# fabioiuri/DRecPy

Hardware: AMD Instinct MI355X
Metric: training samples/sec (user-item pairs) (higher is better)
Workload: dtype f32; 1 GPU; CDAE hidden_factors=128 sampled-output sparse-Adagrad on synth-10m-shaped synthetic (10000000 users x 1000000 items, 199573906 positives), corruption 0.2, neg_ratio 5; batch_per_gpu=65536, global_batch=65536, touch_list=prepared ahead on a side stream, batches=fresh device-sampled batch every step (sampler running ahead on the side stream)

## Files before the change

drecpy_amd/_lib.py:

```python
import ctypes as C
import os

_HERE = os.path.dirname(os.path.abspath(__file__))
LIB_PATH = os.path.join(_HERE, 'libdrx.so')

LOSS_BCE, LOSS_MSE = 0, 1
TARGETS_REFERENCE, TARGETS_PER_ROW = 0, 1
OPT_ADAM, OPT_ADAGRAD, OPT_ROWWISE_ADAGRAD = 0, 1, 2
DENSE_AUX_CLEAN = 0x100
KEY_NONE = 0xFFFFFFFF
SHARD_SELF_BYPASS = 1
BATCH_SHARE_USERS = 1


class DrxError(RuntimeError):
    pass


DRX_REC_SIGMOID_BIAS, DRX_REC_BIAS, DRX_REC_CLIP = 0, 1, 2

KNN_METRICS = {'cosine': 0, 'adjusted_cosine': 1, 'cosine_cf': 2, 'jaccard': 3, 'msd': 4, 'pearson': 5}
KNN_USER, KNN_ITEM = 0, 1
KNN_AGGREGATIONS = {'mean': 0, 'weighted_mean': 1}

# ... 269 lines not shown
    'drx_sampler_create': (C.c_void_p, [C.c_void_p, C.c_void_p, C.c_void_p, C.c_int64, C.c_int32, C.c_int32,
                                        C.c_double, C.c_int64]),
    'drx_sampler_sample': (C.c_int, [C.c_void_p, C.c_int32, C.c_void_p, C.c_void_p, C.c_void_p]),
    'drx_cdae_reference_draw': (C.c_int, [C.c_void_p, C.c_void_p, C.c_void_p, C.c_int64, C.c_uint64, C.c_void_p, C.c_void_p, C.c_int32,
                                          C.c_int32, C.c_double, C.c_void_p, C.c_void_p, C.c_void_p, C.c_void_p, C.c_void_p, C.c_void_p,
                                          C.c_int64]),
    'drx_drawahead_create': (C.c_void_p, [C.c_void_p, C.c_void_p, C.c_void_p, C.c_void_p, C.c_void_p, C.c_int32]),
    'drx_drawahead_submit': (C.c_int64, [C.c_void_p, C.c_int32, C.c_int64, C.c_uint64, C.c_int32, C.c_double, C.c_void_p, C.c_void_p,
                                         C.c_void_p, C.c_void_p, C.c_void_p, C.c_void_p, C.c_int64]),
    'drx_drawahead_wait': (C.c_int, [C.c_void_p, C.c_int32, C.c_int64]),
    'drx_drawahead_destroy': (None, [C.c_void_p]),
    'drx_cdae_fit_slot_bytes': (C.c_size_t, [C.c_int32, C.c_int64]),
    'drx_cdae_fit_dense': (C.c_int, [C.POINTER(CdaeParams), C.POINTER(Optim), C.POINTER(History), C.c_void_p, C.c_void_p, C.c_int32,
                                     C.c_float, C.c_int64, C.c_int32, C.c_int32, C.c_int64, C.c_void_p, C.c_void_p, C.c_size_t,
                                     C.c_int32, C.c_void_p, C.c_size_t, C.c_void_p, C.c_size_t, C.c_void_p]),
    'drx_sampler_draw': (C.c_int, [C.c_void_p, C.c_int32, C.c_int32, C.c_void_p, C.c_void_p, C.c_void_p, C.c_void_p]),
    'drx_sampler_destroy': (None, [C.c_void_p]),
    'drx_cdae_kshard_forward': (C.c_int, [C.POINTER(CdaeParams), C.POINTER(History), C.POINTER(Batch), C.c_void_p, C.c_void_p,
                                          C.c_void_p]),
    'drx_cdae_kshard_forward_prepared': (C.c_int, [C.POINTER(CdaeParams), C.POINTER(History), C.POINTER(Batch), C.c_void_p, C.c_size_t, C.c_void_p,
                                                   C.c_void_p, C.c_void_p]),
    'drx_cdae_kshard_step': (C.c_int, [C.POINTER(CdaeParams), C.POINTER(Optim), C.POINTER(History), C.POINTER(Batch), C.c_int32,
                                       C.c_void_p, C.c_void_p, C.c_void_p, C.c_size_t, C.c_void_p, C.c_size_t, C.c_void_p,
                                       C.c_void_p, C.c_void_p]),
    'drx_cdae_prep_result_bytes': (C.c_size_t, [C.POINTER(CdaeParams), C.c_int32, C.c_int32]),
    'drx_cdae_prep_part_out_bytes': (C.c_size_t, [C.POINTER(CdaeParams), C.c_int32, C.c_int32, C.c_int32]),
    'drx_cdae_prep_part_layout': (C.c_int, [C.POINTER(CdaeParams), C.c_int32, C.c_int32, C.c_int32, C.POINTER(C.c_size_t)]),
    'drx_cdae_prep_part_bytes': (C.c_size_t, [C.POINTER(CdaeParams), C.c_int32, C.c_int32, C.c_int32]),
    'drx_cdae_sparse_prepare_part': (C.c_int, [C.POINTER(CdaeParams), C.POINTER(History), C.POINTER(Batch), C.c_int32, C.c_int32,
                                               C.c_void_p, C.c_size_t, C.c_void_p, C.c_size_t, C.c_void_p]),
    'drx_cdae_sparse_prepare_assemble': (C.c_int, [C.POINTER(CdaeParams), C.POINTER(Batch), C.c_void_p, C.c_int32, C.c_void_p,
                                                   C.c_size_t, C.c_void_p, C.c_void_p]),
    'drx_sort_pairs_temp_bytes': (C.c_size_t, [C.c_int64, C.c_int32]),
    'drx_sort_pairs': (C.c_int, [C.c_void_p, C.c_void_p, C.c_void_p, C.c_void_p, C.c_int64, C.c_int32, C.c_void_p, C.c_size_t, C.c_void_p]),
    'drx_list_sampler_create': (C.c_void_p, [C.c_void_p, C.c_void_p, C.c_void_p, C.c_int32, C.c_int32, C.c_int32, C.c_int32,
                                             C.c_int32, C.c_int32, C.c_int64]),
    'drx_list_sampler_sample': (C.c_int, [C.c_void_p, C.c_int32, C.c_void_p, C.c_void_p, C.c_void_p, C.c_int64, C.c_void_p,
                                          C.c_void_p, C.c_int64, C.c_void_p, C.c_void_p, C.c_int64]),
    'drx_list_sampler_last_hint': (C.c_int32, [C.c_void_p]),
    'drx_list_sampler_destroy': (None, [C.c_void_p]),
    'drx_rng_create': (C.c_void_p, [C.c_int64]),
    'drx_rng_destroy': (None, [C.c_void_p]),
    'drx_rng_random': (C.c_double, [C.c_void_p]),
    'drx_rng_randint': (C.c_int64, [C.c_void_p, C.c_int64, C.c_int64]),
    'drx_rng_discard': (None, [C.c_void_p, C.c_uint64]),
    'drx_rng_corruption_keep': (C.c_int, [C.c_void_p, C.c_void_p, C.c_void_p, C.c_int32, C.c_void_p, C.c_int32,
                                          C.c_double, C.c_void_p, C.c_void_p, C.c_int64]),
}


def batch_offsets(indptr, ids):
    import torch
    B = int(ids.numel())
    off = torch.empty(B + 1, dtype=torch.int32, device=ids.device)
    need = int(lib().drx_point_sample_scratch_bytes(B))
    sc = torch.empty(need, dtype=torch.uint8, device=ids.device)
    check(lib().drx_batch_offsets(ptr(indptr), ptr(ids), B, ptr(off), ptr(sc), need, stream_ptr(ids.device)), 'drx_batch_offsets')
    return off


def sumsq(tensors, device=None):
    import torch
    ts = [t for t in tensors if t is not None and t.numel()]
    if not ts:
        return 0.0
    dev = ts[0].device
# ... 49 lines not shown
```

drecpy_amd/csrc/drx_prep.hpp:

```cpp
#pragma once
#include <algorithm>
#include "drx_common.hpp"
#include "drx_rows.hpp"
#include "drx_segreduce.hpp"
#include "drx_scan.hpp"

namespace drx {

struct WireGeo {
  int ipr, cshift, world;
  __host__ __device__ __forceinline__ uint32_t wire(int item, int is_out) const {
    const int o = item / ipr;
    const uint32_t l = 2u * (uint32_t)(item - o * ipr) + (uint32_t)(is_out ? 1 : 0);
    return (((l >> cshift) * (uint32_t)world + (uint32_t)o) << cshift) | (l & ((1u << cshift) - 1u));
  }
  __host__ __device__ __forceinline__ uint32_t local(uint32_t w) const {
    return (((w >> cshift) / (uint32_t)world) << cshift) | (w & ((1u << cshift) - 1u));
  }
  __host__ __device__ __forceinline__ uint32_t unit(uint32_t w) const { return w >> cshift; }
};

struct TouchPresence {
  uint8_t *present;
  WireGeo G;
  __device__ __forceinline__ uint32_t wire(int item, int is_out) const { return G.wire(item, is_out); }
};

#ifndef DRX_HOT_LDS_LOOKUP
#define DRX_HOT_LDS_LOOKUP 1
#endif
struct HotMark {
  const int16_t *slot;
  uint32_t *mask;
  int H, Bw;
  const int32_t *item;
  int tbits;
};
static inline int hot_table_bits(int H) {
  int b = 0;
  while ((1 << b) < 4 * H) ++b;
  return b;
}
static inline size_t hot_table_lds_bytes(int H) { return H > 0 && DRX_HOT_LDS_LOOKUP ? ((size_t)6 << hot_table_bits(H)) : 0; }
__device__ __forceinline__ uint32_t hot_table_home(int item, int tbits) { return ((uint32_t)item * 2654435761u) >> (32 - tbits); }

static __global__ __launch_bounds__(kBlock) void k_sparse_touches(int n_items, DrxHistory H, DrxBatch bt, uint32_t qthr, uint32_t *keys,
                                                           uint32_t *vals, int T, uint8_t *solo, uint32_t *zero_a,
                                                           int n_zero_a, uint32_t *zero_b, int n_zero_b, uint32_t *zero_c, int n_zero_c,
                                                           TouchPresence pres, HotMark hot) {
  constexpr int G = 16;
  const int lane = threadIdx.x % G;
  const int b = blockIdx.x * (kBlock / G) + threadIdx.x / G;
  for (int w = blockIdx.x * kBlock + threadIdx.x; w < n_zero_a; w += gridDim.x * kBlock) zero_a[w] = 0u;
  for (int w = blockIdx.x * kBlock + threadIdx.x; w < n_zero_b; w += gridDim.x * kBlock) zero_b[w] = 0u;
  for (int w = blockIdx.x * kBlock + threadIdx.x; w < n_zero_c; w += gridDim.x * kBlock) zero_c[w] = 0u;
  __shared__ uint32_t hm[DRX_MAX_HOT];
  extern __shared__ __align__(16) int hot_table[];
  const uint32_t tmask = (1u << hot.tbits) - 1u;
  uint16_t *const hot_slot_of = reinterpret_cast<uint16_t *>(hot_table + tmask + 1);
  if (hot.slot) {
    for (int i = threadIdx.x; i < hot.H; i += kBlock) hm[i] = 0u;
    if (DRX_HOT_LDS_LOOKUP) {
      for (int i = threadIdx.x; i <= (int)tmask; i += kBlock) hot_table[i] = -1;
      __syncthreads();
      for (int i = threadIdx.x; i < hot.H; i += kBlock) {
        const int it = hot.item[i];
        uint32_t at = hot_table_home(it, hot.tbits);
        while (atomicCAS(&hot_table[at], -1, it) != -1) at = (at + 1u) & tmask;
        hot_slot_of[at] = (uint16_t)i;
      }
    }
    __syncthreads();
  }
  if (b < bt.B) {
  if (solo && lane == 0) { solo[b] = 0; solo[bt.B + b] = 0; }
  if (b == bt.B - 1)
    for (int j = bt.keep_off[bt.B] + 2 * bt.B + lane; j < T; j += G) { keys[j] = DRX_KEY_NONE; vals[j] = 0; }
  const int u = bt.uid[b];
  const int64_t s = H.indptr[u], e = H.indptr[u + 1];
  const int base = bt.keep_off[b] + 2 * b;
  const uint8_t *kp = bt.keep ? bt.keep + bt.keep_off[b] : nullptr;
  for (int64_t j = s + lane; j < e; j += G) {
    const uint32_t jj = (uint32_t)(j - s);
    const bool kf = kp ? (kp[jj] != 0) : (hash_u32(bt.mask_seed, (uint32_t)b, jj) >= qthr);
    const int item = H.indices[j];
    int hs = -1;
    if (hot.slot && kf) {
      if (DRX_HOT_LDS_LOOKUP) {
        for (uint32_t at = hot_table_home(item, hot.tbits);; at = (at + 1u) & tmask) {
          const int k = hot_table[at];
          if (k == item) hs = (int)hot_slot_of[at];
          if (k == item || k == -1) break;
        }
      } else hs = (int)hot.slot[item];
    }
    keys[base + jj] = kf && hs < 0 ? (uint32_t)item : DRX_KEY_NONE;
    vals[base + jj] = (uint32_t)b;
    if (hs >= 0) atomicOr(&hm[hs], 1u << (b & 15));
    if (pres.present && kf) pres.present[pres.wire(item, 0)] = 1;
  }
  if (lane == 0) {
    const int deg = (int)(e - s);
    keys[base + deg] = (uint32_t)(n_items + bt.iid[b]);       vals[base + deg] = (uint32_t)b;
    if (pres.present) pres.present[pres.wire(bt.iid[b], 1)] = 1;
    keys[base + deg + 1] = (uint32_t)(2 * n_items) + (uint32_t)u;       vals[base + deg + 1] = (uint32_t)b;
  }
  }
  if (hot.slot) {
    __syncthreads();
    uint16_t *const m16 = reinterpret_cast<uint16_t *>(hot.mask);
    const size_t row = 2 * (size_t)hot.Bw;
    const bool tail = blockIdx.x + 1 == gridDim.x && blockIdx.x + 1 < row;
    for (int i = threadIdx.x; i < hot.H; i += kBlock) {
      m16[(size_t)i * row + blockIdx.x] = (uint16_t)hm[i];
      if (tail) m16[(size_t)i * row + blockIdx.x + 1] = 0;
    }
  }
}

static __global__ __launch_bounds__(1024) void k_degree_counts(const int32_t *__restrict__ keep_off, int B, unsigned int *__restrict__ work) {
  __shared__ unsigned int cnt[256];
  degree_counts_body<1024>(keep_off, B, work, (int)blockIdx.x, cnt);
}

template <int NT>
__device__ __forceinline__ void degree_scatter_body(const int32_t *__restrict__ keep_off, int B, unsigned int *__restrict__ work,
                                                    int32_t *__restrict__ order, int block_id, unsigned int *lds ) {
  unsigned int *start = lds, *cnt = lds + 256, *base = lds + 512;
  for (int i = threadIdx.x; i < 256; i += NT) cnt[i] = 0;
  if (threadIdx.x < 64) {
    unsigned int c[4], sum = 0;
#pragma unroll
    for (int q = 0; q < 4; ++q) { c[q] = work[threadIdx.x * 4 + q]; sum += c[q]; }
    unsigned int inc = sum;
#pragma unroll
    for (int o = 1; o < 64; o <<= 1) { const unsigned int t = __shfl_up(inc, o); if ((int)threadIdx.x >= o) inc += t; }
    unsigned int run = inc - sum;
#pragma unroll
    for (int q = 0; q < 4; ++q) { start[threadIdx.x * 4 + q] = run; run += c[q]; }
  }
  __syncthreads();
  const int b = block_id * NT + (int)threadIdx.x, lane = threadIdx.x & 63;
  const bool valid = b < B;
  const int d = valid ? degree_bucket(keep_off, b) : 0;
  const unsigned long long m = same_bucket_lanes(valid, d);
  const int leader = valid ? __ffsll((long long)m) - 1 : lane;
  unsigned int at = 0;
  if (valid && lane == leader) at = atomicAdd(&cnt[d], (unsigned int)__popcll(m));
// ... 478 lines not shown
                     R.order_work, 512);
  int rc = sort_pairs(stemp, sb, k2, ks, v2, vs, (size_t)2 * B, bits2, st);
  if (rc) return rc;
  hipLaunchKernelGGL(k_tp_runs, dim3((2 * B + 255) / 256 < 1024 ? (2 * B + 255) / 256 : 1024), dim3(256), 0, st, ks, 2 * B, start, end);
  const int egrid = U < (1 << 20) ? U : (1 << 20);
  const int wgrid = (int)((nnz + 255) / 256 < 16384 ? (nnz + 255) / 256 : 16384);
  const int rt = share_item_triples(p->ld);
  if (share) {
    const int ig = (B + 255) / 256;
    hipLaunchKernelGGL(k_tp_item_flags, dim3(ig), dim3(256), 0, st, ks, B, rt, start, R.pitem, R.n_du);
    rc = scan_i32(sctemp2, scb2, R.pitem, R.pitem, (size_t)B, true, st);
    if (rc) return rc;
    hipLaunchKernelGGL(k_tp_item_finish, dim3(ig), dim3(256), 0, st, ks, vs, B, rt, start, end, hist->indptr, R.usamp, R.pitem, R.witem,
                       R.n_du, R.plan.cnt);
    hipLaunchKernelGGL(k_tp_item_order, dim3(ig), dim3(256), 0, st, ks, B, rt, start, hist->indptr, R.pitem, R.worder, R.n_du);
    hipLaunchKernelGGL((k_tp_count<true>), dim3(egrid), dim3(256), 0, st, *hist, *bt, qthr, U, start, end, vs, cnt, km, rt);
  } else
    hipLaunchKernelGGL((k_tp_count<false>), dim3(egrid), dim3(256), 0, st, *hist, *bt, qthr, U, start, end, vs, cnt, km, rt);
  int *cnt_last = (int *)R.vals;
  DRX_HIP(hipMemcpyAsync(cnt_last, cnt + (nnz - 1), sizeof(int), hipMemcpyDeviceToDevice, st));
  rc = scan_i32(sctemp, scb, cnt, cnt, (size_t)nnz, false, st);
  if (rc) return rc;
  if (share)
    hipLaunchKernelGGL((k_tp_write<true>), dim3(wgrid), dim3(256), 0, st, *hist, *bt, qthr, start, end, vs, cnt, km, R.keys_s, R.vals_s, R.pitem, rt, row_end);
  else
    hipLaunchKernelGGL((k_tp_write<false>), dim3(wgrid), dim3(256), 0, st, *hist, *bt, qthr, start, end, vs, cnt, km, R.keys_s, R.vals_s, R.pitem, rt, row_end);
  hipLaunchKernelGGL(k_tp_tail, dim3(2048), dim3(256), 0, st, ks, vs, B, U, N, cnt + (nnz - 1), cnt_last, R.T, R.keys_s, R.vals_s, R.plan.cnt);
  return DRX_OK;
}

static int prepare_impl(const DrxCdaeParams *p, const DrxHistory *hist, const DrxBatch *bt, const PrepBufs &R, hipStream_t st,
                        bool with_marks = false, TouchPresence pres = TouchPresence{nullptr, WireGeo{1, 0, 1}},
                        const int16_t *hot_slot = nullptr, const int32_t *hot_item = nullptr) {
  const int gpb = kBlock / 16;
  if (R.H > 0 && (!hot_slot || !hot_item || !hot_list_fits(R.T, *p, pres.present != nullptr))) return DRX_EINVAL;
  if (hist->t_rank && hist->t_users && hist->t_pos && hist->t_items && !pres.present && long_segments(R.T, *p)) {
    const int32_t *row_end = nullptr;
    const int rc = prepare_transposed(p, hist, bt, R, st, with_marks, &row_end);
    if (rc == DRX_OK) {
      PrepBufs Rb = R;
      Rb.plan.row_end = row_end;
      Rb.plan.row_end_keys = (uint32_t)p->n_items;
      if (with_marks && p->ld > 16) {
        if (!share_users(p, hist, bt, R)) order_by_degree(bt, R, st, true);
        const int blocks = std::max(2048, (R.n_chunks + 255) / 256);
        hipLaunchKernelGGL(k_plan_and_mark, dim3(blocks), dim3(256), 0, st, R.keys_s, R.vals_s, R.T, R.n_chunks,
                           kSegBlock / pick_geom(p->ld).G, Rb.plan, (uint32_t)p->n_items, bt->B, R.solo_v, R.solo_o, 0, bt->keep_off,
                           R.order_work, R.order);
        if (R.plan.xrank) hipLaunchKernelGGL(k_place_blocks, dim3(256), dim3(256), 0, st, Rb.plan, R.n_chunks);
        return DRX_OK;
      }
      return plan_spans(p, bt, Rb, st, true);
    }
    if (rc != kTpFallback) return rc;
  }
  uint32_t *sort_zero = nullptr;
  size_t sort_zero_words = 0;
  sort_pairs_zero_region(R.sort_temp, (size_t)R.T, R.bits, &sort_zero, &sort_zero_words);
  hipLaunchKernelGGL(k_sparse_touches, dim3((bt->B + gpb - 1) / gpb), dim3(kBlock), hot_table_lds_bytes(R.H), st, p->n_items, *hist, *bt,
                     q_threshold(bt->q), R.keys, R.vals, R.T, R.solo_v, R.plan.cnt, plan_zero_words(R), R.order_work, 512,
                     sort_zero, (int)sort_zero_words, pres, HotMark{R.H > 0 ? hot_slot : nullptr, R.hmask, R.H, R.Bw, hot_item, hot_table_bits(R.H)});
  const bool fused_order = with_marks && p->ld > 16;
  const SortRider rider{fused_order ? bt->keep_off : nullptr, bt->B, R.order_work};
  const int rc = sort_pairs_ex(R.sort_temp, R.sort_bytes, R.keys, R.keys_s, R.vals, R.vals_s, (size_t)R.T, R.bits, true, st, true, rider);
  if (rc) return rc;
  if (with_marks && p->ld > 16) {
    const int blocks = std::max(2048, (R.n_chunks + 255) / 256);
    const int order_blocks = (bt->B + 255) / 256;
    hipLaunchKernelGGL(k_plan_and_mark, dim3(blocks + order_blocks), dim3(256), 0, st, R.keys_s, R.vals_s, R.T, R.n_chunks,
                       kSegBlock / pick_geom(p->ld).G, R.plan, (uint32_t)p->n_items, bt->B, R.solo_v, R.solo_o,
                       order_blocks, bt->keep_off, R.order_work, R.order);
    if (R.plan.xrank) hipLaunchKernelGGL(k_place_blocks, dim3(256), dim3(256), 0, st, R.plan, R.n_chunks);
    return DRX_OK;
  }
  return plan_spans(p, bt, R, st, true);
}

static int mark_solo(const DrxCdaeParams *p, const DrxBatch *bt, const PrepBufs &R, hipStream_t st, bool cleared) {
  if (!cleared) {
    DRX_HIP(hipMemsetAsync(R.solo_v, 0, (size_t)bt->B * 2, st));
  }
  if (p->ld <= 16) return DRX_OK;
  hipLaunchKernelGGL(k_mark_solo, dim3(2048), dim3(256), 0, st, R.keys_s, R.vals_s, R.T, (uint32_t)p->n_items, bt->B, R.solo_v,
                     R.solo_o);
  return DRX_OK;
}


}
```

drecpy_amd/csrc/drx_sort.hip:

```cpp
#include <cstdlib>
#include <cstring>
#include <hip/hip_runtime.h>
#include "drx_common.hpp"

namespace drx {

#ifndef DRX_SORT_THREADS
#define DRX_SORT_THREADS 512
#endif
#ifndef DRX_SORT_IPT
#define DRX_SORT_IPT 16
#endif
constexpr int kSortThreads = DRX_SORT_THREADS;
constexpr int kSortWaves = kSortThreads / 64;
constexpr int kSortIPT = DRX_SORT_IPT;
constexpr int kSortTile = kSortThreads * kSortIPT;
constexpr int kMaxPasses = 4;
constexpr uint32_t kStAgg = 1u << 30, kStIncl = 2u << 30, kCountMask = (1u << 30) - 1;
constexpr int kDropNone = 1, kFirstPass = 2, kLastPass = 4;

struct SortPlan {
  int passes;
  int rbits[kMaxPasses];
  int shift[kMaxPasses];
};

inline SortPlan sort_plan(int bits) {
  SortPlan p{};
  int passes = (bits + 10) / 11;
  if (bits <= 8) passes = 1;
  int r = (bits + passes - 1) / passes;
  if (r < 8 && bits >= 8) r = 8;
  if (r <= 8) r = 8; else if (r <= 10) r = 10; else r = 11;
  p.passes = (bits + r - 1) / r;
  for (int i = 0; i < p.passes; ++i) { p.rbits[i] = r; p.shift[i] = i * r; }
  return p;
}

struct SortLayout {
  uint32_t *tmp_k, *tmp_v;
  uint32_t *hist;
  uint32_t *ticket;
  uint32_t *desc;
  size_t zero_begin, zero_bytes;
  size_t total;
  int tiles;
};

inline SortLayout sort_layout(void *temp, size_t n, const SortPlan &P) {
  SortLayout L{};
  Carver cv(temp, (size_t)-1);
  L.tiles = (int)((n + kSortTile - 1) / kSortTile);
  if (P.passes >= 2) { L.tmp_k = cv.take<uint32_t>(n); L.tmp_v = cv.take<uint32_t>(n); }
  cv.off = align_up(cv.off, 256);
  L.zero_begin = cv.off;
  L.hist = cv.take<uint32_t>((size_t)kMaxPasses * 2048);
  L.ticket = cv.take<uint32_t>(64);
  size_t d = 0;
  for (int i = 0; i < P.passes; ++i) d += (size_t)L.tiles << P.rbits[i];
  L.desc = cv.take<uint32_t>(d);
  L.zero_bytes = cv.off - L.zero_begin;
  L.total = align_up(cv.off, 256);
  return L;
}

__global__ __launch_bounds__(512) void k_digit_histograms(const uint32_t *__restrict__ keys, size_t n, SortPlan P, uint32_t *__restrict__ hist,
                                                          int drop_none, SortRider rider, int rider_blocks) {
  __shared__ uint32_t h[kMaxPasses * 2048];
  if ((int)blockIdx.x >= (int)gridDim.x - rider_blocks) {
    degree_counts_body<512>(rider.keep_off, rider.B, rider.counts, (int)blockIdx.x - ((int)gridDim.x - rider_blocks), h);
    return;
  }
  const size_t hist_threads = (size_t)((int)gridDim.x - rider_blocks) * blockDim.x;
  for (int i = threadIdx.x; i < P.passes * 2048; i += blockDim.x) h[i] = 0;
  __syncthreads();
  const uint32_t lane = threadIdx.x & 63;
  for (size_t i = (size_t)blockIdx.x * blockDim.x + threadIdx.x; i < n; i += hist_threads) {
    const uint32_t k = keys[i];
    if (drop_none && k == DRX_KEY_NONE) continue;
    for (int p = 0; p < P.passes; ++p) {
      const uint32_t rep_bits = 11u - (uint32_t)P.rbits[p];
      const uint32_t d = (k >> P.shift[p]) & ((1u << P.rbits[p]) - 1);
      atomicAdd(&h[p * 2048 + (d << rep_bits) + (lane & ((1u << rep_bits) - 1u))], 1u);
    }
  }
  __syncthreads();
  for (int p = 0; p < P.passes; ++p) {
    const uint32_t rep_bits = 11u - (uint32_t)P.rbits[p], reps = 1u << rep_bits;
    for (uint32_t d = threadIdx.x; d < (1u << P.rbits[p]); d += blockDim.x) {
      uint32_t c = 0;
      for (uint32_t r = 0; r < reps; ++r) c += h[p * 2048 + (d << rep_bits) + r];
      if (c) atomicAdd(&hist[p * 2048 + d], c);
    }
  }
}

template <int R>
__global__ __launch_bounds__(kSortThreads) void k_onesweep_pass(const uint32_t *__restrict__ kin, const uint32_t *__restrict__ vin,
                                                               uint32_t *__restrict__ kout, uint32_t *__restrict__ vout, size_t n, int shift,
                                                               const uint32_t *__restrict__ ghist, uint32_t *ticket, uint32_t *desc, uint32_t n_tiles,
                                                               int flags, uint32_t *next_hist, int next_shift) {
  constexpr int RADIX = 1 << R;
  constexpr int BPT = (RADIX + kSortThreads - 1) / kSortThreads;
  extern __shared__ __align__(16) uint32_t sort_lds[];
  uint32_t (*whist)[RADIX] = reinterpret_cast<uint32_t (*)[RADIX]>(sort_lds);
  uint32_t *gbase = sort_lds + kSortWaves * RADIX;
  uint32_t *lstart = gbase + RADIX;
  uint32_t *skey = lstart + RADIX, *sval = skey + kSortTile;
  constexpr int REPB = 11 - R, REP = 1 << REPB;
  uint32_t *nh = sval + kSortTile;
  __shared__ uint32_t s_tile, s_tile_valid;
  __shared__ uint32_t wl[kSortWaves], wg[kSortWaves];
  const int tid = threadIdx.x, lane = tid & 63, w = tid >> 6;
  const bool drop = flags & kDropNone, first = flags & kFirstPass, last = flags & kLastPass;
  size_t n_valid = n;
  if (drop) {
    uint32_t part = 0;
    for (int d = tid; d < RADIX; d += kSortThreads) part += ghist[d];
#pragma unroll
    for (int o = 32; o > 0; o >>= 1) part += __shfl_xor(part, o);
    if (lane == 0) wl[w] = part;
    __syncthreads();
    uint32_t tot = 0;
    for (int ww = 0; ww < kSortWaves; ++ww) tot += wl[ww];
    n_valid = tot;
    __syncthreads();
// ... 72 lines not shown
    __syncthreads();
#pragma unroll
    for (int q = 0; q < BPT; ++q) { const int d = tid * BPT + q; if (d < RADIX) local[q] = lstart[d]; sl += local[q]; }
    __syncthreads();
    uint32_t il = sl, ig = sg;
#pragma unroll
    for (int o = 1; o < 64; o <<= 1) {
      const uint32_t tl = __shfl_up(il, o), tg = __shfl_up(ig, o);
      if (lane >= o) { il += tl; ig += tg; }
    }
    if (lane == 63) { wl[w] = il; wg[w] = ig; }
    __syncthreads();
    uint32_t ol = il - sl, og = ig - sg;
    for (int ww = 0; ww < w; ++ww) { ol += wl[ww]; og += wg[ww]; }
#pragma unroll
    for (int q = 0; q < BPT; ++q) {
      const int d = tid * BPT + q;
      if (d < RADIX) { lstart[d] = ol; gbase[d] = og; }
      ol += local[q]; og += glob[q];
      if (d == RADIX - 1) s_tile_valid = ol;
    }
  }
  __syncthreads();

#pragma unroll
  for (int q = 0; q < BPT; ++q) {
    const int d = tid + q * kSortThreads;
    excl[q] = 0;
    if (d < RADIX && tile > 0) {
      uint32_t sum = 0;
      int p = (int)tile - 1;
      bool done = false;
      while (!done) {
        uint32_t wv[8];
#pragma unroll
        for (int u = 0; u < 8; ++u)
          wv[u] = (p - u >= 0) ? __hip_atomic_load(desc + ((size_t)(p - u) << R) + d, __ATOMIC_RELAXED, __HIP_MEMORY_SCOPE_AGENT) : kStIncl;
#pragma unroll
        for (int u = 0; u < 8; ++u) {
          if (done) break;
          uint32_t x = wv[u];
          while ((x >> 30) == 0) {
            __builtin_amdgcn_s_sleep(1);
            x = __hip_atomic_load(desc + ((size_t)(p - u) << R) + d, __ATOMIC_RELAXED, __HIP_MEMORY_SCOPE_AGENT);
          }
          sum += x & kCountMask;
          if ((x >> 30) == 2u) done = true;
        }
        p -= 8;
      }
      excl[q] = sum;
      __hip_atomic_store(desc + ((size_t)tile << R) + d, kStIncl | (sum + cnt[q]), __ATOMIC_RELAXED, __HIP_MEMORY_SCOPE_AGENT);
    }
  }
#pragma unroll
  for (int q = 0; q < BPT; ++q) {
    const int d = tid + q * kSortThreads;
    if (d < RADIX) gbase[d] = gbase[d] + excl[q] - lstart[d];
  }
#pragma unroll
  for (int it = 0; it < kSortIPT; ++it) {
    const int idx = w * (64 * kSortIPT) + it * 64 + lane;
    if (idx < tile_n && !(drop && key[it] == DRX_KEY_NONE)) {
      const uint32_t d = (key[it] >> shift) & (RADIX - 1);
      const uint32_t pos = lstart[d] + whist[w][d] + pre[it];
      skey[pos] = key[it];
      sval[pos] = val[it];
    }
  }
  __syncthreads();
  const int tile_out = (int)s_tile_valid;
  for (int i = tid; i < tile_out; i += kSortThreads) {
    const uint32_t k = skey[i];
    const uint32_t d = (k >> shift) & (RADIX - 1);
    const size_t o = (size_t)gbase[d] + (size_t)i;
    kout[o] = k;
    vout[o] = sval[i];
  }
  }
  if (next_hist) {
    for (int d = tid; d < RADIX; d += kSortThreads) {
      uint32_t c = 0;
// ... 17 lines not shown
static int launch_pass(const uint32_t *sk, const uint32_t *sv, uint32_t *dk, uint32_t *dv, size_t n, int shift, const uint32_t *gh, uint32_t *ticket,
                       uint32_t *desc, int tiles, int flags, uint32_t *next_hist, int next_shift, hipStream_t stream) {
  const size_t lds = onesweep_lds_bytes(R);
  if (lds > 48 * 1024) DRX_HIP(hipFuncSetAttribute((const void *)k_onesweep_pass<R>, hipFuncAttributeMaxDynamicSharedMemorySize, (int)lds));
  hipLaunchKernelGGL(k_onesweep_pass<R>, dim3(tiles < sort_grid() ? tiles : sort_grid()), dim3(kSortThreads), lds, stream, sk, sv, dk, dv, n, shift, gh,
                     ticket, desc, (uint32_t)tiles, flags, next_hist, next_shift);
  return 0;
}

size_t sort_pairs_temp_bytes(size_t n, int end_bit) {
  const SortPlan P = sort_plan(end_bit);
  return sort_layout(nullptr, n ? n : 1, P).total + 256;
}

void sort_pairs_zero_region(void *temp, size_t n, int end_bit, uint32_t **words, size_t *n_words) {
  const SortPlan P = sort_plan(end_bit);
  char *t = (char *)align_up((size_t)temp, 256);
  const SortLayout L = sort_layout(t, n ? n : 1, P);
  *words = (uint32_t *)(t + L.zero_begin);
  *n_words = L.zero_bytes / 4;
}

int sort_pairs_ex(void *temp, size_t temp_bytes, const uint32_t *kin, uint32_t *kout, const uint32_t *vin, uint32_t *vout, size_t n, int end_bit,
                  bool drop_none, hipStream_t stream, bool pre_zeroed, SortRider rider) {
  if (n == 0) return 0;
  if (n >= (1u << 30)) return DRX_EINVAL;
  const SortPlan P = sort_plan(end_bit);
  char *t = (char *)align_up((size_t)temp, 256);
  const SortLayout L = sort_layout(t, n, P);
  if ((size_t)(t - (char *)temp) + L.total > temp_bytes) return DRX_ESCRATCH;
  if (!pre_zeroed) DRX_HIP(hipMemsetAsync(t + L.zero_begin, 0, L.zero_bytes, stream));
  int hgrid = (int)((n + 8 * 512 - 1) / (8 * 512));
  if (hgrid > sort_grid()) hgrid = sort_grid();
  SortPlan P1 = P;
  P1.passes = 1;
  const int rider_blocks = rider.keep_off ? (rider.B + 511) / 512 : 0;
  hipLaunchKernelGGL(k_digit_histograms, dim3(hgrid + rider_blocks), dim3(512), 0, stream, kin, n, P1, L.hist, drop_none ? 1 : 0, rider,
                     rider_blocks);
  const uint32_t *src_k = kin, *src_v = vin;
  uint32_t *desc = L.desc;
  for (int p = 0; p < P.passes; ++p) {
    const bool to_out = ((P.passes - 1 - p) & 1) == 0;
    uint32_t *dk = to_out ? kout : L.tmp_k, *dv = to_out ? vout : L.tmp_v;
    const uint32_t *gh = L.hist + (size_t)p * 2048;
    const int flags = (drop_none ? kDropNone : 0) | (p == 0 ? kFirstPass : 0) | (p == P.passes - 1 ? kLastPass : 0);
    int rc;
    uint32_t *nh = p + 1 < P.passes ? L.hist + (size_t)(p + 1) * 2048 : nullptr;
    const int ns = p + 1 < P.passes ? P.shift[p + 1] : 0;
    if (P.rbits[p] == 8) rc = launch_pass<8>(src_k, src_v, dk, dv, n, P.shift[p], gh, L.ticket + p, desc, L.tiles, flags, nh, ns, stream);
    else if (P.rbits[p] == 10) rc = launch_pass<10>(src_k, src_v, dk, dv, n, P.shift[p], gh, L.ticket + p, desc, L.tiles, flags, nh, ns, stream);
    else rc = launch_pass<11>(src_k, src_v, dk, dv, n, P.shift[p], gh, L.ticket + p, desc, L.tiles, flags, nh, ns, stream);
    if (rc) return rc;
    desc += (size_t)L.tiles << P.rbits[p];
    src_k = dk; src_v = dv;
  }
  DRX_LAUNCH_CHECK();
  return 0;
}

int sort_pairs(void *temp, size_t temp_bytes, const uint32_t *kin, uint32_t *kout, const uint32_t *vin,
               uint32_t *vout, size_t n, int end_bit, hipStream_t stream) {
  return sort_pairs_ex(temp, temp_bytes, kin, kout, vin, vout, n, end_bit, false, stream);
}

}

extern "C" {
size_t drx_sort_pairs_temp_bytes(int64_t n, int32_t key_bits) {
  if (n < 0 || key_bits < 1 || key_bits > 32) return 0;
  return drx::sort_pairs_temp_bytes((size_t)n, key_bits) + 256;
}
int drx_sort_pairs(const uint32_t *keys_in, uint32_t *keys_out, const uint32_t *vals_in, uint32_t *vals_out, int64_t n, int32_t key_bits,
                   void *temp, size_t temp_bytes, void *stream) {
  if (n < 0 || key_bits < 1 || key_bits > 32 || (n > 0 && (!keys_in || !keys_out || !vals_in || !vals_out || !temp))) return DRX_EINVAL;
  return drx::sort_pairs(temp, temp_bytes, keys_in, keys_out, vals_in, vals_out, (size_t)n, key_bits, (hipStream_t)stream);
}
}
```

include/drx.h:

```cpp
#ifndef DRX_H_
#define DRX_H_

#include <stddef.h>
#include <stdint.h>

#ifdef __cplusplus
extern "C" {
#endif

#define DRX_VERSION 100

enum {
  DRX_OK = 0,
  DRX_EINVAL = -1,
  DRX_ESCRATCH = -2,
  DRX_ENOTIMPL = -3,
  DRX_ERETRY = -4,
  DRX_ECOMM = -5
};

#define DRX_MAX_K 1024
#define DRX_KEY_NONE 0xFFFFFFFFu

enum { DRX_LOSS_BCE = 0, DRX_LOSS_MSE = 1 };
// ... 400 lines not shown

int drx_rows_pair_scores(const float *table, const float *bias, int32_t n_rows, int32_t ld, int32_t epilogue,
                         const float *q, int32_t n_q, const int32_t *q_row, const int32_t *t_row, int64_t P,
                         float *out_score, void *stream);

#define DRX_KNN_COSINE          0
#define DRX_KNN_ADJUSTED_COSINE 1
#define DRX_KNN_COSINE_CF       2
#define DRX_KNN_JACCARD         3
#define DRX_KNN_MSD             4
#define DRX_KNN_PEARSON         5
#define DRX_KNN_USER            0
#define DRX_KNN_ITEM            1
#define DRX_KNN_MEAN            0
#define DRX_KNN_WEIGHTED_MEAN   1
size_t drx_knn_neighbours_scratch_bytes(int32_t R, int32_t C, int32_t k, int32_t splits);
int drx_knn_neighbours(const int64_t *indptr, const int32_t *indices, const float *values, int64_t nnz, int32_t R, int32_t C,
                       int32_t metric, int32_t k, int32_t m, double shrinkage, double max_diff, int32_t splits,
                       int32_t *out_idx, float *out_sim, void *scratch, size_t scratch_bytes, void *stream);

int drx_knn_row_means(const int64_t *indptr, const float *values, int64_t nnz, int32_t R, double *out_mean, void *stream);

size_t drx_knn_score_rows_scratch_bytes(int32_t type, int32_t R, int32_t n_items);
int drx_knn_score_rows(int32_t type, int32_t aggregation, const int64_t *indptr, const int32_t *indices, const float *values, int64_t nnz,
                       int32_t n_users, int32_t n_items, const int32_t *nb_idx, const float *nb_sim, int32_t k,
                       const int32_t *uid, int32_t R, const double *fallback, float *out, uint32_t *cand_mask,
                       void *scratch, size_t scratch_bytes, void *stream);
int drx_knn_pair_scores(int32_t type, int32_t aggregation, const int64_t *indptr, const int32_t *indices, const float *values, int64_t nnz,
                        int32_t n_users, int32_t n_items, const int32_t *nb_idx, const float *nb_sim, int32_t k,
                        const int32_t *uid, const int32_t *iid, int64_t P, const double *fallback, double *out, uint8_t *none,
                        void *stream);

size_t drx_sort_pairs_temp_bytes(int64_t n, int32_t key_bits);
int drx_sort_pairs(const uint32_t *keys_in, uint32_t *keys_out, const uint32_t *vals_in, uint32_t *vals_out, int64_t n, int32_t key_bits,
                   void *temp, size_t temp_bytes, void *stream);

size_t drx_idmap_scratch_bytes(int64_t n);
int drx_idmap_build(const int64_t *raw, int64_t n, int32_t *codes, int64_t *uniques,
                    int32_t *n_unique, void *scratch, size_t scratch_bytes, void *stream);

typedef struct DrxSampler DrxSampler;
DrxSampler *drx_sampler_create(const int32_t *h_uid, const int32_t *h_iid, const double *h_val, int64_t n_rows,
                               int32_t neg_ratio, int32_t has_threshold, double threshold, int64_t seed);
int drx_sampler_sample(DrxSampler *s, int32_t n, int32_t *h_uid_out, int32_t *h_iid_out, double *h_val_out);
enum { DRX_DRAW_MIXED = 0, DRX_DRAW_NEGATIVE = 1, DRX_DRAW_POSITIVE = 2 };
int drx_sampler_draw(DrxSampler *s, int32_t kind, int32_t n, int32_t *h_uid_out, int32_t *h_iid_out, double *h_val_out,
                     uint8_t *h_neg_out);
void drx_sampler_destroy(DrxSampler *s);

typedef struct DrxListSampler DrxListSampler;
DrxListSampler *drx_list_sampler_create(const int64_t *grp_indptr, const int64_t *grp_rows, const int32_t *grp_ids, int32_t n_groups,
                                        int32_t n_ids, int32_t neg_ratio, int32_t n_targets, int32_t min_positive,
                                        int32_t max_positive, int64_t seed);
int drx_list_sampler_sample(DrxListSampler *s, int32_t n, int32_t *group_out, int64_t *in_off, int64_t *in_rows, int64_t in_cap,
                            int64_t *tg_off, int64_t *tg_rows, int64_t tg_cap, int64_t *ng_off, int32_t *neg_ids, int64_t ng_cap);
int32_t drx_list_sampler_last_hint(const DrxListSampler *s);
void drx_list_sampler_destroy(DrxListSampler *s);

typedef struct DrxRng DrxRng;
DrxRng *drx_rng_create(int64_t seed);
void drx_rng_destroy(DrxRng *r);
double drx_rng_random(DrxRng *r);
int64_t drx_rng_randint(DrxRng *r, int64_t a, int64_t b);
void drx_rng_discard(DrxRng *r, uint64_t n_words);
int drx_rng_corruption_keep(DrxRng *r, const int64_t *h_indptr, const int32_t *h_indices, int32_t n_items,
                            const int32_t *h_uid, int32_t B, double q,
// ... 27 lines not shown
```

Baseline: 208.1 million samples/s.

## Batch touch kernel over many samples per block and simplify sort histogram

The touch-list kernel now handles 128 samples per block in several rounds instead of 16. It prefetches uids, degrees and the first history indices into registers, and keeps a multi-word hot-item bitmask per block that is written out as full 32-bit words rather than 16-bit chunks. This cuts per-block hot-table setup and mask traffic, but raises LDS use, which may now need the dynamic shared memory attribute, and lowers the block count. The sort histogram kernel is specialized to a single pass with a fixed 2048-entry LDS array, the lookback depth becomes a tunable constant, and a geometry query entry point is added.

```diff
diff --git a/drecpy_amd/_lib.py b/drecpy_amd/_lib.py
--- a/drecpy_amd/_lib.py
+++ b/drecpy_amd/_lib.py
@@ -325,6 +325,7 @@
     'drx_cdae_sparse_prepare_assemble': (C.c_int, [C.POINTER(CdaeParams), C.POINTER(Batch), C.c_void_p, C.c_int32, C.c_void_p,
                                                    C.c_size_t, C.c_void_p, C.c_void_p]),
     'drx_sort_pairs_temp_bytes': (C.c_size_t, [C.c_int64, C.c_int32]),
+    'drx_sort_geometry': (None, [C.POINTER(C.c_int32), C.POINTER(C.c_int32), C.POINTER(C.c_int32)]),
     'drx_sort_pairs': (C.c_int, [C.c_void_p, C.c_void_p, C.c_void_p, C.c_void_p, C.c_int64, C.c_int32, C.c_void_p, C.c_size_t, C.c_void_p]),
     'drx_list_sampler_create': (C.c_void_p, [C.c_void_p, C.c_void_p, C.c_void_p, C.c_int32, C.c_int32, C.c_int32, C.c_int32,
                                              C.c_int32, C.c_int32, C.c_int64]),
diff --git a/drecpy_amd/csrc/drx_prep.hpp b/drecpy_amd/csrc/drx_prep.hpp
--- a/drecpy_amd/csrc/drx_prep.hpp
+++ b/drecpy_amd/csrc/drx_prep.hpp
@@ -29,6 +29,15 @@
 #ifndef DRX_HOT_LDS_LOOKUP
 #define DRX_HOT_LDS_LOOKUP 1
 #endif
+#ifndef DRX_TOUCH_SAMPLES
+#define DRX_TOUCH_SAMPLES 128
+#endif
+constexpr int kTouchSamples = DRX_TOUCH_SAMPLES;
+constexpr int kTouchGroup = 16;
+constexpr int kTouchRounds = kTouchSamples / (kBlock / kTouchGroup);
+constexpr int kTouchWords = kTouchSamples / 32;
+constexpr int kTouchAhead = 2;
+static_assert(kTouchSamples % 32 == 0 && kTouchSamples % (kBlock / kTouchGroup) == 0, "whole mask words, whole rounds");
 struct HotMark {
   const int16_t *slot;
   uint32_t *mask;
@@ -41,25 +50,32 @@
   while ((1 << b) < 4 * H) ++b;
   return b;
 }
-static inline size_t hot_table_lds_bytes(int H) { return H > 0 && DRX_HOT_LDS_LOOKUP ? ((size_t)6 << hot_table_bits(H)) : 0; }
+static inline size_t hot_table_lds_bytes(int H) {
+  return H > 0 ? (size_t)H * kTouchWords * 4 + (DRX_HOT_LDS_LOOKUP ? ((size_t)6 << hot_table_bits(H)) : 0) : 0;
+}
 __device__ __forceinline__ uint32_t hot_table_home(int item, int tbits) { return ((uint32_t)item * 2654435761u) >> (32 - tbits); }
 
 static __global__ __launch_bounds__(kBlock) void k_sparse_touches(int n_items, DrxHistory H, DrxBatch bt, uint32_t qthr, uint32_t *keys,
                                                            uint32_t *vals, int T, uint8_t *solo, uint32_t *zero_a,
                                                            int n_zero_a, uint32_t *zero_b, int n_zero_b, uint32_t *zero_c, int n_zero_c,
                                                            TouchPresence pres, HotMark hot) {
-  constexpr int G = 16;
+  constexpr int G = kTouchGroup, GPB = kBlock / G;
   const int lane = threadIdx.x % G;
-  const int b = blockIdx.x * (kBlock / G) + threadIdx.x / G;
+  const int b0 = blockIdx.x * kTouchSamples + threadIdx.x / G;
   for (int w = blockIdx.x * kBlock + threadIdx.x; w < n_zero_a; w += gridDim.x * kBlock) zero_a[w] = 0u;
   for (int w = blockIdx.x * kBlock + threadIdx.x; w < n_zero_b; w += gridDim.x * kBlock) zero_b[w] = 0u;
   for (int w = blockIdx.x * kBlock + threadIdx.x; w < n_zero_c; w += gridDim.x * kBlock) zero_c[w] = 0u;
-  __shared__ uint32_t hm[DRX_MAX_HOT];
-  extern __shared__ __align__(16) int hot_table[];
+  int u[kTouchRounds], deg[kTouchRounds], base[kTouchRounds], ahead[kTouchRounds][kTouchAhead];
+  int64_t s[kTouchRounds];
+#pragma unroll
+  for (int r = 0; r < kTouchRounds; ++r) u[r] = b0 + r * GPB < bt.B ? bt.uid[b0 + r * GPB] : 0;
+  extern __shared__ __align__(16) int touch_lds[];
+  uint32_t *const hm = reinterpret_cast<uint32_t *>(touch_lds);
+  int *const hot_table = touch_lds + (hot.slot ? hot.H * kTouchWords : 0);
   const uint32_t tmask = (1u << hot.tbits) - 1u;
   uint16_t *const hot_slot_of = reinterpret_cast<uint16_t *>(hot_table + tmask + 1);
   if (hot.slot) {
-    for (int i = threadIdx.x; i < hot.H; i += kBlock) hm[i] = 0u;
+    for (int i = threadIdx.x; i < hot.H * kTouchWords; i += kBlock) hm[i] = 0u;
     if (DRX_HOT_LDS_LOOKUP) {
       for (int i = threadIdx.x; i <= (int)tmask; i += kBlock) hot_table[i] = -1;
       __syncthreads();
@@ -72,48 +88,60 @@
     }
     __syncthreads();
   }
-  if (b < bt.B) {
-  if (solo && lane == 0) { solo[b] = 0; solo[bt.B + b] = 0; }
-  if (b == bt.B - 1)
-    for (int j = bt.keep_off[bt.B] + 2 * bt.B + lane; j < T; j += G) { keys[j] = DRX_KEY_NONE; vals[j] = 0; }
-  const int u = bt.uid[b];
-  const int64_t s = H.indptr[u], e = H.indptr[u + 1];
-  const int base = bt.keep_off[b] + 2 * b;
-  const uint8_t *kp = bt.keep ? bt.keep + bt.keep_off[b] : nullptr;
-  for (int64_t j = s + lane; j < e; j += G) {
-    const uint32_t jj = (uint32_t)(j - s);
-    const bool kf = kp ? (kp[jj] != 0) : (hash_u32(bt.mask_seed, (uint32_t)b, jj) >= qthr);
-    const int item = H.indices[j];
-    int hs = -1;
-    if (hot.slot && kf) {
-      if (DRX_HOT_LDS_LOOKUP) {
-        for (uint32_t at = hot_table_home(item, hot.tbits);; at = (at + 1u) & tmask) {
-          const int k = hot_table[at];
-          if (k == item) hs = (int)hot_slot_of[at];
-          if (k == item || k == -1) break;
-        }
-      } else hs = (int)hot.slot[item];
-    }
-    keys[base + jj] = kf && hs < 0 ? (uint32_t)item : DRX_KEY_NONE;
-    vals[base + jj] = (uint32_t)b;
-    if (hs >= 0) atomicOr(&hm[hs], 1u << (b & 15));
-    if (pres.present && kf) pres.present[pres.wire(item, 0)] = 1;
-  }
-  if (lane == 0) {
-    const int deg = (int)(e - s);
-    keys[base + deg] = (uint32_t)(n_items + bt.iid[b]);       vals[base + deg] = (uint32_t)b;
-    if (pres.present) pres.present[pres.wire(bt.iid[b], 1)] = 1;
-    keys[base + deg + 1] = (uint32_t)(2 * n_items) + (uint32_t)u;       vals[base + deg + 1] = (uint32_t)b;
-  }
+#pragma unroll
+  for (int r = 0; r < kTouchRounds; ++r) {
+    const bool live = b0 + r * GPB < bt.B;
+    s[r] = live ? H.indptr[u[r]] : 0;
+    deg[r] = live ? (int)(H.indptr[u[r] + 1] - s[r]) : 0;
+    base[r] = live ? bt.keep_off[b0 + r * GPB] + 2 * (b0 + r * GPB) : 0;
+  }
+#pragma unroll
+  for (int r = 0; r < kTouchRounds; ++r)
+#pragma unroll
+    for (int a = 0; a < kTouchAhead; ++a) ahead[r][a] = lane + a * G < deg[r] ? H.indices[s[r] + lane + a * G] : 0;
+#pragma unroll
+  for (int r = 0; r < kTouchRounds; ++r) {
+    const int b = b0 + r * GPB;
+    if (b >= bt.B) continue;
+    if (solo && lane == 0) { solo[b] = 0; solo[bt.B + b] = 0; }
+    if (b == bt.B - 1)
+      for (int j = bt.keep_off[bt.B] + 2 * bt.B + lane; j < T; j += G) { keys[j] = DRX_KEY_NONE; vals[j] = 0; }
+    const uint8_t *kp = bt.keep ? bt.keep + (base[r] - 2 * b) : nullptr;
+    const uint32_t bit = 1u << (b & 31);
+    uint32_t *const hrow = hm + (threadIdx.x / G + r * GPB) / 32;
+    for (int jj = lane, a = 0; jj < deg[r]; jj += G, ++a) {
+      const bool kf = kp ? (kp[jj] != 0) : (hash_u32(bt.mask_seed, (uint32_t)b, (uint32_t)jj) >= qthr);
+      int item;
+      if (a == 0) item = ahead[r][0];
+      else if (a == 1) item = ahead[r][1];
+      else item = H.indices[s[r] + jj];
+      int hs = -1;
+      if (hot.slot && kf) {
+        if (DRX_HOT_LDS_LOOKUP) {
+          for (uint32_t at = hot_table_home(item, hot.tbits);; at = (at + 1u) & tmask) {
+            const int k = hot_table[at];
+            if (k == item) hs = (int)hot_slot_of[at];
+            if (k == item || k == -1) break;
+          }
+        } else hs = (int)hot.slot[item];
+      }
+      keys[base[r] + jj] = kf && hs < 0 ? (uint32_t)item : DRX_KEY_NONE;
+      vals[base[r] + jj] = (uint32_t)b;
+      if (hs >= 0) atomicOr(&hrow[hs * kTouchWords], bit);
+      if (pres.present && kf) pres.present[pres.wire(item, 0)] = 1;
+    }
+    if (lane == 0) {
+      keys[base[r] + deg[r]] = (uint32_t)(n_items + bt.iid[b]);       vals[base[r] + deg[r]] = (uint32_t)b;
+      if (pres.present) pres.present[pres.wire(bt.iid[b], 1)] = 1;
+      keys[base[r] + deg[r] + 1] = (uint32_t)(2 * n_items) + (uint32_t)u[r];       vals[base[r] + deg[r] + 1] = (uint32_t)b;
+    }
   }
   if (hot.slot) {
     __syncthreads();
-    uint16_t *const m16 = reinterpret_cast<uint16_t *>(hot.mask);
-    const size_t row = 2 * (size_t)hot.Bw;
-    const bool tail = blockIdx.x + 1 == gridDim.x && blockIdx.x + 1 < row;
-    for (int i = threadIdx.x; i < hot.H; i += kBlock) {
-      m16[(size_t)i * row + blockIdx.x] = (uint16_t)hm[i];
-      if (tail) m16[(size_t)i * row + blockIdx.x + 1] = 0;
+    const int w0 = blockIdx.x * kTouchWords;
+    for (int i = threadIdx.x; i < hot.H * kTouchWords; i += kBlock) {
+      const int w = w0 + i % kTouchWords;
+      if (w < hot.Bw) hot.mask[(size_t)(i / kTouchWords) * hot.Bw + w] = hm[i];
     }
   }
 }
@@ -658,7 +686,6 @@
 static int prepare_impl(const DrxCdaeParams *p, const DrxHistory *hist, const DrxBatch *bt, const PrepBufs &R, hipStream_t st,
                         bool with_marks = false, TouchPresence pres = TouchPresence{nullptr, WireGeo{1, 0, 1}},
                         const int16_t *hot_slot = nullptr, const int32_t *hot_item = nullptr) {
-  const int gpb = kBlock / 16;
   if (R.H > 0 && (!hot_slot || !hot_item || !hot_list_fits(R.T, *p, pres.present != nullptr))) return DRX_EINVAL;
   if (hist->t_rank && hist->t_users && hist->t_pos && hist->t_items && !pres.present && long_segments(R.T, *p)) {
     const int32_t *row_end = nullptr;
@@ -683,7 +710,9 @@
   uint32_t *sort_zero = nullptr;
   size_t sort_zero_words = 0;
   sort_pairs_zero_region(R.sort_temp, (size_t)R.T, R.bits, &sort_zero, &sort_zero_words);
-  hipLaunchKernelGGL(k_sparse_touches, dim3((bt->B + gpb - 1) / gpb), dim3(kBlock), hot_table_lds_bytes(R.H), st, p->n_items, *hist, *bt,
+  if (hot_table_lds_bytes(R.H) > 48 * 1024)
+    DRX_HIP(hipFuncSetAttribute((const void *)k_sparse_touches, hipFuncAttributeMaxDynamicSharedMemorySize, (int)hot_table_lds_bytes(R.H)));
+  hipLaunchKernelGGL(k_sparse_touches, dim3((bt->B + kTouchSamples - 1) / kTouchSamples), dim3(kBlock), hot_table_lds_bytes(R.H), st, p->n_items, *hist, *bt,
                      q_threshold(bt->q), R.keys, R.vals, R.T, R.solo_v, R.plan.cnt, plan_zero_words(R), R.order_work, 512,
                      sort_zero, (int)sort_zero_words, pres, HotMark{R.H > 0 ? hot_slot : nullptr, R.hmask, R.H, R.Bw, hot_item, hot_table_bits(R.H)});
   const bool fused_order = with_marks && p->ld > 16;
diff --git a/drecpy_amd/csrc/drx_sort.hip b/drecpy_amd/csrc/drx_sort.hip
--- a/drecpy_amd/csrc/drx_sort.hip
+++ b/drecpy_amd/csrc/drx_sort.hip
@@ -16,6 +16,10 @@
 constexpr int kSortIPT = DRX_SORT_IPT;
 constexpr int kSortTile = kSortThreads * kSortIPT;
 constexpr int kMaxPasses = 4;
+#ifndef DRX_SORT_LOOKBACK
+#define DRX_SORT_LOOKBACK 8
+#endif
+constexpr int kSortLookback = DRX_SORT_LOOKBACK;
 constexpr uint32_t kStAgg = 1u << 30, kStIncl = 2u << 30, kCountMask = (1u << 30) - 1;
 constexpr int kDropNone = 1, kFirstPass = 2, kLastPass = 4;
 
@@ -64,34 +68,29 @@
   return L;
 }
 
-__global__ __launch_bounds__(512) void k_digit_histograms(const uint32_t *__restrict__ keys, size_t n, SortPlan P, uint32_t *__restrict__ hist,
-                                                          int drop_none, SortRider rider, int rider_blocks) {
-  __shared__ uint32_t h[kMaxPasses * 2048];
+__global__ __launch_bounds__(512) void k_digit_histograms(const uint32_t *__restrict__ keys, size_t n, int rbits, int shift,
+                                                          uint32_t *__restrict__ hist, int drop_none, SortRider rider, int rider_blocks) {
+  __shared__ uint32_t h[2048];
   if ((int)blockIdx.x >= (int)gridDim.x - rider_blocks) {
     degree_counts_body<512>(rider.keep_off, rider.B, rider.counts, (int)blockIdx.x - ((int)gridDim.x - rider_blocks), h);
     return;
   }
   const size_t hist_threads = (size_t)((int)gridDim.x - rider_blocks) * blockDim.x;
-  for (int i = threadIdx.x; i < P.passes * 2048; i += blockDim.x) h[i] = 0;
+  for (int i = threadIdx.x; i < 2048; i += blockDim.x) h[i] = 0;
   __syncthreads();
   const uint32_t lane = threadIdx.x & 63;
+  const uint32_t rep_bits = 11u - (uint32_t)rbits, reps = 1u << rep_bits;
   for (size_t i = (size_t)blockIdx.x * blockDim.x + threadIdx.x; i < n; i += hist_threads) {
     const uint32_t k = keys[i];
     if (drop_none && k == DRX_KEY_NONE) continue;
-    for (int p = 0; p < P.passes; ++p) {
-      const uint32_t rep_bits = 11u - (uint32_t)P.rbits[p];
-      const uint32_t d = (k >> P.shift[p]) & ((1u << P.rbits[p]) - 1);
-      atomicAdd(&h[p * 2048 + (d << rep_bits) + (lane & ((1u << rep_bits) - 1u))], 1u);
-    }
-  }
-  __syncthreads();
-  for (int p = 0; p < P.passes; ++p) {
-    const uint32_t rep_bits = 11u - (uint32_t)P.rbits[p], reps = 1u << rep_bits;
-    for (uint32_t d = threadIdx.x; d < (1u << P.rbits[p]); d += blockDim.x) {
-      uint32_t c = 0;
-      for (uint32_t r = 0; r < reps; ++r) c += h[p * 2048 + (d << rep_bits) + r];
-      if (c) atomicAdd(&hist[p * 2048 + d], c);
-    }
+    const uint32_t d = (k >> shift) & ((1u << rbits) - 1);
+    atomicAdd(&h[(d << rep_bits) + (lane & (reps - 1u))], 1u);
+  }
+  __syncthreads();
+  for (uint32_t d = threadIdx.x; d < (1u << rbits); d += blockDim.x) {
+    uint32_t c = 0;
+    for (uint32_t r = 0; r < reps; ++r) c += h[(d << rep_bits) + r];
+    if (c) atomicAdd(&hist[d], c);
   }
 }
 
@@ -230,12 +229,12 @@
       int p = (int)tile - 1;
       bool done = false;
       while (!done) {
-        uint32_t wv[8];
-#pragma unroll
-        for (int u = 0; u < 8; ++u)
+        uint32_t wv[kSortLookback];
+#pragma unroll
+        for (int u = 0; u < kSortLookback; ++u)
           wv[u] = (p - u >= 0) ? __hip_atomic_load(desc + ((size_t)(p - u) << R) + d, __ATOMIC_RELAXED, __HIP_MEMORY_SCOPE_AGENT) : kStIncl;
 #pragma unroll
-        for (int u = 0; u < 8; ++u) {
+        for (int u = 0; u < kSortLookback; ++u) {
           if (done) break;
           uint32_t x = wv[u];
           while ((x >> 30) == 0) {
@@ -245,7 +244,7 @@
           sum += x & kCountMask;
           if ((x >> 30) == 2u) done = true;
         }
-        p -= 8;
+        p -= kSortLookback;
       }
       excl[q] = sum;
       __hip_atomic_store(desc + ((size_t)tile << R) + d, kStIncl | (sum + cnt[q]), __ATOMIC_RELAXED, __HIP_MEMORY_SCOPE_AGENT);
@@ -329,10 +328,8 @@
   if (!pre_zeroed) DRX_HIP(hipMemsetAsync(t + L.zero_begin, 0, L.zero_bytes, stream));
   int hgrid = (int)((n + 8 * 512 - 1) / (8 * 512));
   if (hgrid > sort_grid()) hgrid = sort_grid();
-  SortPlan P1 = P;
-  P1.passes = 1;
   const int rider_blocks = rider.keep_off ? (rider.B + 511) / 512 : 0;
-  hipLaunchKernelGGL(k_digit_histograms, dim3(hgrid + rider_blocks), dim3(512), 0, stream, kin, n, P1, L.hist, drop_none ? 1 : 0, rider,
+  hipLaunchKernelGGL(k_digit_histograms, dim3(hgrid + rider_blocks), dim3(512), 0, stream, kin, n, P.rbits[0], P.shift[0], L.hist, drop_none ? 1 : 0, rider,
                      rider_blocks);
   const uint32_t *src_k = kin, *src_v = vin;
   uint32_t *desc = L.desc;
@@ -367,6 +364,11 @@
   if (n < 0 || key_bits < 1 || key_bits > 32) return 0;
   return drx::sort_pairs_temp_bytes((size_t)n, key_bits) + 256;
 }
+void drx_sort_geometry(int32_t *tile_pairs, int32_t *lookback, int32_t *grid_cap) {
+  if (tile_pairs) *tile_pairs = drx::kSortTile;
+  if (lookback) *lookback = drx::kSortLookback;
+  if (grid_cap) *grid_cap = drx::sort_grid();
+}
 int drx_sort_pairs(const uint32_t *keys_in, uint32_t *keys_out, const uint32_t *vals_in, uint32_t *vals_out, int64_t n, int32_t key_bits,
                    void *temp, size_t temp_bytes, void *stream) {
   if (n < 0 || key_bits < 1 || key_bits > 32 || (n > 0 && (!keys_in || !keys_out || !vals_in || !vals_out || !temp))) return DRX_EINVAL;
diff --git a/include/drx.h b/include/drx.h
--- a/include/drx.h
+++ b/include/drx.h
@@ -456,6 +456,7 @@
                         void *stream);
 
 size_t drx_sort_pairs_temp_bytes(int64_t n, int32_t key_bits);
+void drx_sort_geometry(int32_t *tile_pairs, int32_t *lookback, int32_t *grid_cap);
 int drx_sort_pairs(const uint32_t *keys_in, uint32_t *keys_out, const uint32_t *vals_in, uint32_t *vals_out, int64_t n, int32_t key_bits,
                    void *temp, size_t temp_bytes, void *stream);
 
```

After: 210.4 million samples/s, median of 3. Within noise of the previous version (+1.1%).
